# symek/facedeform

Hardware: AMD Instinct MI355X
Metric: deformed Mverts/sec at 256 ctrl pts, 1/2/4/8 MI355X vs host-CPU ref (higher is better)
Workload: dtype f32

## Files before the change

### facedeform_amd/csrc/fd_build_reg.hip

```cpp
#include <cstdio>
#include <cstdlib>

#include "fd_internal.h"
#include "fd_pack.h"

namespace fd {

namespace {

typedef double double4_t __attribute__((ext_vector_type(4)));

constexpr double kEps = 2.220446049250313e-16;
constexpr int kRegThreads = 512;
constexpr int kRegWaves = kRegThreads / 64;
constexpr int kMaxBlocks = 16;
constexpr int kWorkers = 7;
constexpr int kSlots = 20;
constexpr int kPitch = 17;
constexpr int kTileLds = 16 * kPitch;

__device__ __forceinline__ double readlane_f64(double v, int src_lane)
{
    const long long b = __double_as_longlong(v);
    const unsigned lo = (unsigned)__builtin_amdgcn_readlane((int)(b & 0xffffffffll), src_lane);
// ... 52 lines not shown
    return fma(y0, p, y0);
}

__device__ __forceinline__ double log_pos(double x)
{
    double m = __builtin_amdgcn_frexp_mant(x);
    int e = __builtin_amdgcn_frexp_exp(x);
    if (m < 0.70710678118654752) { m *= 2.0; e -= 1; }
    const double num = m - 1.0, den = m + 1.0;
    double r = __builtin_amdgcn_rcp(den);
    r = fma(fma(-den, r, 1.0), r, r);
    r = fma(fma(-den, r, 1.0), r, r);
    double s0 = num * r;
    s0 = fma(fma(-den, s0, num), r, s0);
    const double z = s0 * s0;
    double p = 1.0 / 21.0;
    p = fma(p, z, 1.0 / 19.0);
    p = fma(p, z, 1.0 / 17.0);
    p = fma(p, z, 1.0 / 15.0);
    p = fma(p, z, 1.0 / 13.0);
    p = fma(p, z, 1.0 / 11.0);
    p = fma(p, z, 1.0 / 9.0);
    p = fma(p, z, 1.0 / 7.0);
    p = fma(p, z, 1.0 / 5.0);
    p = fma(p, z, 1.0 / 3.0);
    const double lnm = fma(s0 * z, 2.0 * p, 2.0 * s0);
    return fma((double)e, 0.69314718055994530942, lnm);
}
__device__ __forceinline__ double phi_reg(int kind, double d2, double inv_r2)
{
    switch (kind) {
    case FD_KERNEL_GAUSSIAN: return exp(-d2 * inv_r2);
    case FD_KERNEL_THIN_PLATE: return d2 > 0.0 ? 0.5 * d2 * log_pos(d2) : 0.0;
    case FD_KERNEL_BIHARMONIC: return -sqrt(d2);
    default: return d2 * sqrt(d2);
    }
}

struct RegLds {
    double *cen, *V, *W, *F, *B21, *small, *minv, *P, *scr, *Z, *Y, *stat, *ypart, *D;
    int *tab, *flag;
};
constexpr int kSmallDoubles = 96;
constexpr int kTau = 0, kR = 4, kTm = 20, kG = 36, kGm = 48;
constexpr int kRows = 16 * kMaxBlocks;
__host__ __device__ inline size_t reg_lds_doubles(int)
{
    const size_t overlay = (size_t)kMaxBlocks * kTileLds + (size_t)(kMaxBlocks + 1) * kTileLds;
    const size_t ypart = (size_t)kRegWaves * 4 * kRows;
    return (size_t)3 * kRows + 4 * (size_t)kRows + 4 * (size_t)kRows + 3 * (size_t)kRows + 4 * (size_t)kRows + kSmallDoubles +
           (overlay > ypart ? overlay : ypart) + (size_t)kRegWaves * 2 * kTileLds + 3 * 256 + 3 * 256 + 8 + kTileLds + 160 ;
}
__device__ __forceinline__ RegLds carve(double *base, int)
{
    RegLds L;
    double *p = base;
    L.cen = p; p += 3 * kRows;
    L.V = p; p += 4 * kRows;
    L.W = p; p += 4 * kRows;
    L.F = p; p += 3 * kRows;
    L.B21 = p; p += 4 * kRows;
    L.small = p; p += kSmallDoubles;
    const size_t overlay = (size_t)kMaxBlocks * kTileLds + (size_t)(kMaxBlocks + 1) * kTileLds;
    const size_t ypart = (size_t)kRegWaves * 4 * kRows;
    L.minv = p; L.P = p + (size_t)kMaxBlocks * kTileLds; L.ypart = p;
    p += overlay > ypart ? overlay : ypart;
    L.scr = p; p += (size_t)kRegWaves * 2 * kTileLds;
    L.Z = p; p += 3 * 256;
    L.Y = p; p += 3 * 256;
    L.stat = p; p += 8;
    L.D = p; p += kTileLds;
    L.tab = reinterpret_cast<int *>(p);
    L.flag = L.tab + 300;
    return L;
}

__device__ __forceinline__ double4_t factor_invert_tile(double4_t Tt, int lane, double &piv)
{
    const int c = lane & 15, g = lane >> 4;
    piv = 0.0;
    double4_t U;
#pragma unroll
    for (int i = 0; i < 4; ++i) U[i] = (g + 4 * i == c) ? 1.0 : 0.0;
#pragma unroll
    for (int b = 0; b < 4; ++b) {
        double s[4][4];
#pragma unroll
        for (int p = 0; p < 4; ++p)
#pragma unroll
            for (int q = 0; q <= p; ++q) s[p][q] = readlane_f64(Tt[b], 4 * b + q + 16 * p);
        double l[4][4], inv[4], dk[4];
#pragma unroll
        for (int k = 0; k < 4; ++k) {
            double d = s[k][k];
#pragma unroll
            for (int e = 0; e < k; ++e) d = fma(-l[k][e], l[k][e], d);
            dk[k] = d;
            inv[k] = rsqrt_nr(d);
#pragma unroll
            for (int p = k + 1; p < 4; ++p) {
                double v = s[p][k];
#pragma unroll
                for (int e = 0; e < k; ++e) v = fma(-l[p][e], l[k][e], v);
                l[p][k] = v * inv[k];
            }
        }
#pragma unroll
        for (int k = 0; k < 4; ++k) piv = c == 4 * b + k ? dk[k] : piv;
        double m[4][4];
#pragma unroll
        for (int q = 0; q < 4; ++q) {
            m[q][q] = inv[q];
#pragma unroll
            for (int p = q + 1; p < 4; ++p) {
                double v = 0.0;
#pragma unroll
                for (int e = q; e < p; ++e) v = fma(l[p][e], m[e][q], v);
                m[p][q] = -v * inv[p];
            }
        }
        double aop = 0.0;
#pragma unroll
        for (int p = 0; p < 4; ++p)
#pragma unroll
            for (int q = 0; q <= p; ++q) aop = (c == p && g == q) ? m[p][q] : aop;
        const double4_t zero = {0.0, 0.0, 0.0, 0.0};
        const double4_t rt = __builtin_amdgcn_mfma_f64_16x16x4f64(aop, Tt[b], zero, 0, 0, 0);
        const double4_t ru = __builtin_amdgcn_mfma_f64_16x16x4f64(aop, U[b], zero, 0, 0, 0);
        const double mult = c > 4 * b + 3 ? -rt[0] : 0.0;
        Tt = __builtin_amdgcn_mfma_f64_16x16x4f64(mult, rt[0], Tt, 0, 0, 0);
        U = __builtin_amdgcn_mfma_f64_16x16x4f64(mult, ru[0], U, 0, 0, 0);
        U[b] = ru[0];
        Tt[b] = rt[0];
    }
    return U;
}

constexpr int kAff = 64;
struct PackLds {
    const double *cen, *dlt, *sol, *aff;
    const float *dl_global;
    double R;
    int sing, dup;
    __device__ __forceinline__ double centre(int j, int q) const { return cen[3 * j + q]; }
    __device__ __forceinline__ bool has_delta() const { return true; }
    __device__ __forceinline__ double delta(int j, int q) const { return dlt ? dlt[3 * j + q] : (double)dl_global[3 * j + q]; }
    __device__ __forceinline__ double weight(int j, int c) const { return sol[c * 256 + j]; }
    __device__ __forceinline__ double affine(int cc, int k, int, int T) const { return k < T ? aff[3 * k + cc] : 0.0; }
    __device__ __forceinline__ double radius(int) const { return R; }
    __device__ __forceinline__ int sing_flag() const { return sing; }
    __device__ __forceinline__ int dup_flag() const { return dup; }
};

__device__ __forceinline__ double lds_where(bool cond, const double *p, int i_true)
{
    const double v = p[cond ? i_true : 0];
    return cond ? v : 0.0;
}

__device__ __forceinline__ void assemble_tile(const double *cen, int I, int J, int c, int g, int M, int kind, double lambda, double inv_r2,
                                              double (&e)[4], double &amax_w, bool &dup)
{
    const int col = 16 * J + c;
    const double cx = cen[3 * col], cy = cen[3 * col + 1], cz = cen[3 * col + 2];
    double d2[4];
#pragma unroll
    for (int i = 0; i < 4; ++i) {
        const int row = 16 * I + g + 4 * i;
        const double dx = cen[3 * row] - cx, dy = cen[3 * row + 1] - cy, dz = cen[3 * row + 2] - cz;
        d2[i] = dx * dx + dy * dy + dz * dz;
    }
    if (kind == FD_KERNEL_THIN_PLATE) {
#pragma unroll
        for (int i = 0; i < 4; ++i) {
            const bool pos = d2[i] > 0.0;
            const double lg = log_pos(pos ? d2[i] : 1.0);
            e[i] = pos ? 0.5 * d2[i] * lg : 0.0;
        }
    } else {
#pragma unroll
        for (int i = 0; i < 4; ++i) e[i] = phi_reg(kind, d2[i], inv_r2);
    }
#pragma unroll
    for (int i = 0; i < 4; ++i) {
        const int row = 16 * I + g + 4 * i;
        const bool real = row < M && col < M;
        if (row == col) e[i] += lambda;
        else if (d2[i] == 0.0 && real) dup = true;
        if (!real) e[i] = 0.0;
        const double ae = fabs(e[i]);
        amax_w = ae > amax_w ? ae : amax_w;
    }
}

__device__ __forceinline__ void reflect_wave(const RegLds &L, int M, int T, int lane)
{
    bool singular = false;
    double cn[4] = {0.0, 0.0, 0.0, 0.0};
    double v[4][4], f[4][3];
#pragma unroll
    for (int q = 0; q < 4; ++q) {
        const int i = lane + 64 * q;
        const bool in = i < M;
        const int ic = in ? i : 0;
        const double p[4] = {1.0, L.cen[3 * ic], L.cen[3 * ic + 1], L.cen[3 * ic + 2]};
#pragma unroll
        for (int t = 0; t < 4; ++t) {
            v[q][t] = (in && t < T) ? p[t] : 0.0;
            if (in) cn[t] = fma(v[q][t], v[q][t], cn[t]);
        }
#pragma unroll
        for (int e = 0; e < 3; ++e) { const double d = L.F[e * kRows + ic]; f[q][e] = in ? d : 0.0; }
    }
#pragma unroll
    for (int t = 0; t < 4; ++t) cn[t] = wave_sum(cn[t]);
#pragma unroll
    for (int k = 0; k < 4; ++k) {
        if (k >= T) break;
        const int piv = M - 1 - k;
        const int pl = __builtin_amdgcn_readfirstlane(piv & 63), pq = __builtin_amdgcn_readfirstlane(piv >> 6);
        double rowv[4], rowf[3];
#define FD_PIVOT_ROW(Q) { _Pragma("unroll") for (int t = 0; t < 4; ++t) rowv[t] = readlane_f64(v[Q][t], pl); \
                          _Pragma("unroll") for (int e = 0; e < 3; ++e) rowf[e] = readlane_f64(f[Q][e], pl); }
        if (pq == 0) FD_PIVOT_ROW(0) else if (pq == 1) FD_PIVOT_ROW(1) else if (pq == 2) FD_PIVOT_ROW(2) else FD_PIVOT_ROW(3)
#undef FD_PIVOT_ROW
        double acc[7] = {0.0, 0.0, 0.0, 0.0, 0.0, 0.0, 0.0};
        double x[4];
#pragma unroll
        for (int q = 0; q < 4; ++q) {
            const int i = lane + 64 * q;
            x[q] = i < piv ? v[q][k] : 0.0;
            if (i < piv) {
                acc[0] = fma(x[q], x[q], acc[0]);
#pragma unroll
                for (int cc = k + 1; cc < 4; ++cc) if (cc < T) acc[cc - k] = fma(x[q], v[q][cc], acc[cc - k]);
#pragma unroll
                for (int e = 0; e < 3; ++e) acc[4 + e] = fma(x[q], f[q][e], acc[4 + e]);
            }
        }
#pragma unroll
        for (int e = 0; e < 7; ++e) acc[e] = wave_sum(acc[e]);
        const double xp = rowv[k];
        const double sigma = acc[0];
        const double norm = sqrt(fma(xp, xp, sigma));
        double beta = xp, tau = 0.0, scale = 0.0;
        if (sigma > 0.0) {
            beta = xp >= 0.0 ? -norm : norm;
            tau = (beta - xp) / beta;
            scale = 1.0 / (xp - beta);
        }
        if (!(norm > 64.0 * (double)M * kEps * sqrt(cn[k]))) singular = true;
        double sc[4] = {0.0, 0.0, 0.0, 0.0}, prow[4] = {0.0, 0.0, 0.0, 0.0}, df[3];
#pragma unroll
        for (int cc = k + 1; cc < 4; ++cc) if (cc < T) { prow[cc] = rowv[cc]; sc[cc] = fma(scale, acc[cc - k], prow[cc]); }
#pragma unroll
        for (int e = 0; e < 3; ++e) df[e] = fma(scale, acc[4 + e], rowf[e]);
#pragma unroll
        for (int q = 0; q < 4; ++q) {
            const int i = lane + 64 * q;
            if (i < piv) {
                const double vv = x[q] * scale;
                v[q][k] = vv;
#pragma unroll
                for (int cc = k + 1; cc < 4; ++cc) if (cc < T) v[q][cc] = fma(-tau * sc[cc], vv, v[q][cc]);
#pragma unroll
                for (int e = 0; e < 3; ++e) f[q][e] = fma(-tau * df[e], vv, f[q][e]);
            } else if (i == piv) {
                v[q][k] = 1.0;
#pragma unroll
                for (int cc = k + 1; cc < 4; ++cc) if (cc < T) v[q][cc] = 0.0;
#pragma unroll
                for (int e = 0; e < 3; ++e) f[q][e] = 0.0;
            }
        }
        if (lane == 0) {
            L.small[kTau + k] = tau;
            L.small[kR + 4 * k + k] = beta;
#pragma unroll
            for (int cc = k + 1; cc < 4; ++cc) if (cc < T) L.small[kR + 4 * k + cc] = fma(-tau, sc[cc], prow[cc]);
#pragma unroll
            for (int e = 0; e < 3; ++e) L.small[kG + 3 * k + e] = fma(-tau, df[e], rowf[e]);
        }
    }
#pragma unroll
    for (int q = 0; q < 4; ++q) {
        const int i = lane + 64 * q;
#pragma unroll
        for (int t = 0; t < 4; ++t) L.V[4 * i + t] = v[q][t];
#pragma unroll
        for (int e = 0; e < 3; ++e) L.F[e * kRows + i] = f[q][e];
    }
    wave_lds_sync();
    double gram[6] = {0.0, 0.0, 0.0, 0.0, 0.0, 0.0};
#pragma unroll
    for (int q = 0; q < 4; ++q) {
        const int i = lane + 64 * q;
        if (i < M) {
            const double v0 = v[q][0], v1 = v[q][1], v2 = v[q][2], v3 = v[q][3];
            gram[0] = fma(v0, v1, gram[0]); gram[1] = fma(v0, v2, gram[1]); gram[2] = fma(v0, v3, gram[2]);
            gram[3] = fma(v1, v2, gram[3]); gram[4] = fma(v1, v3, gram[4]); gram[5] = fma(v2, v3, gram[5]);
        }
    }
#pragma unroll
    for (int e = 0; e < 6; ++e) gram[e] = wave_sum(gram[e]);
    {
        const double G[4][4] = {{0.0, gram[0], gram[1], gram[2]}, {0.0, 0.0, gram[3], gram[4]}, {0.0, 0.0, 0.0, gram[5]}, {0.0, 0.0, 0.0, 0.0}};
// ... 730 lines not shown
            L.stat[0] = piv_min; L.stat[1] = piv_max;
            if (bad) L.stat[2] = 1.0;
        }
    }
    FD_RSTAMP()

    auto solve_block = [&](int I) {
        if (lane < 48) {
            const int rhs = lane >> 4, n = lane & 15;
            const double *mi = L.minv + (size_t)I * kTileLds;
            double y = 0.0;
#pragma unroll
            for (int k = 0; k < 16; ++k) y = fma(L.Z[rhs * 256 + 16 * I + k], mi[k * kPitch + n], y);
            L.Y[rhs * 256 + 16 * I + n] = y;
        }
    };
    if (!worker && nb > 0) solve_block(nb - 1);
    __syncthreads();
    if (fac != nullptr && blockIdx.z == 0) {
        gdouble *fg = as_global(fac);
#pragma unroll
        for (int t = 0; t < kSlots; ++t) {
            if (FD_SLOT(m_matrix, t)) {
                const int q = __builtin_amdgcn_readlane(ijv, t) >> 16;
#pragma unroll
                for (int i = 0; i < 4; ++i) fg[kFacL + ((size_t)q * 4 + i) * 64 + lane] = S[t][i];
            }
        }
        for (int e = tid; e < kMaxBlocks * kTileLds; e += kRegThreads) fg[kFacMinv + e] = e < nb * kTileLds ? L.minv[e] : 0.0;
        for (int e = tid; e < 4 * kRows; e += kRegThreads) { fg[kFacV + e] = L.V[e]; fg[kFacB21 + e] = L.B21[e]; }
        if (tid < kSmallDoubles) fg[kFacSmall + tid] = L.small[tid];
        if (tid == 0) {
            fg[kFacMeta + 0] = amax; fg[kFacMeta + 1] = dup_any ? 1.0 : 0.0;
            fg[kFacMeta + 2] = (L.stat[2] != 0.0 || L.stat[3] != 0.0) ? 1.0 : 0.0;
            fg[kFacMeta + 3] = L.stat[0]; fg[kFacMeta + 4] = L.stat[1];
        }
    }
    for (int I = nb - 1; I >= 1; --I) {
        const unsigned m_row = slots_where(ivI == I && ivJ < I);
        const bool next_mine = slots_where(ivI == I && ivJ == I - 1) != 0u;
#pragma unroll
        for (int t = 0; t < kSlots; ++t) {
            if (FD_SLOT(m_row, t)) {
                double4_t acc = {0.0, 0.0, 0.0, 0.0};
                double ya[4];
#pragma unroll
                for (int s = 0; s < 4; ++s) ya[s] = lds_where(c < 3, L.Y, c * 256 + 16 * I + 4 * s + g);
                __builtin_amdgcn_sched_group_barrier(0x100, 4, 0);
                __builtin_amdgcn_sched_group_barrier(0x002, 8, 0);
                __builtin_amdgcn_sched_group_barrier(0x008, 4, 0);
#pragma unroll
                for (int s = 0; s < 4; ++s) acc = __builtin_amdgcn_mfma_f64_16x16x4f64(ya[s], S[t][s], acc, 0, 0, 0);
                if (g < 3) L.Z[g * 256 + 16 * tJ(t) + c] -= acc[0];
            }
        }
        if (next_mine) { wave_lds_sync(); solve_block(I - 1); }
        __syncthreads();
    }
    FD_RSTAMP()

    if (!worker) {
        double q12[12];
#pragma unroll
        for (int e = 0; e < 12; ++e) q12[e] = 0.0;
        double xr[4][3];
#pragma unroll
        for (int q = 0; q < 4; ++q) {
            const int i = lane + 64 * q;
            const bool in = i < n1;
            xr[q][0] = in ? L.Y[i] : 0.0; xr[q][1] = in ? L.Y[256 + i] : 0.0; xr[q][2] = in ? L.Y[512 + i] : 0.0;
            if (in && T > 0) {
#pragma unroll
                for (int k = 0; k < 4; ++k) {
                    const double b = k < T ? L.B21[4 * i + k] : 0.0;
                    q12[3 * k] = fma(b, xr[q][0], q12[3 * k]); q12[3 * k + 1] = fma(b, xr[q][1], q12[3 * k + 1]); q12[3 * k + 2] = fma(b, xr[q][2], q12[3 * k + 2]);
                }
            }
        }
        if (T > 0) {
#pragma unroll
            for (int e = 0; e < 12; ++e) q12[e] = wave_sum(q12[e]);
        }
        double a[4][3] = {};
#pragma unroll
        for (int k = 3; k >= 0; --k) {
            if (k >= T) continue;
#pragma unroll
            for (int e = 0; e < 3; ++e) {
                double v = L.small[kG + 3 * k + e] - q12[3 * k + e];
#pragma unroll
                for (int c2 = k + 1; c2 < 4; ++c2) if (c2 < T) v = fma(-L.small[kR + 4 * k + c2], a[c2][e], v);
                a[k][e] = v / L.small[kR + 4 * k + k];
            }
        }
#pragma unroll
        for (int k = 3; k >= 0; --k) {
            if (k >= T) continue;
            const int piv = M - 1 - k;
            const double tau = L.small[kTau + k];
            double d[3] = {0.0, 0.0, 0.0}, v[4];
#pragma unroll
            for (int q = 0; q < 4; ++q) {
                const int i = lane + 64 * q;
                v[q] = i <= piv ? L.V[4 * i + k] : 0.0;
#pragma unroll
                for (int e = 0; e < 3; ++e) d[e] = fma(v[q], xr[q][e], d[e]);
            }
#pragma unroll
            for (int e = 0; e < 3; ++e) d[e] = wave_sum(d[e]);
#pragma unroll
            for (int q = 0; q < 4; ++q)
#pragma unroll
                for (int e = 0; e < 3; ++e) xr[q][e] = fma(-tau * d[e], v[q], xr[q][e]);
        }
        gdouble *X = as_global(slot.X);
#pragma unroll
        for (int q = 0; q < 4; ++q) {
            const int i = lane + 64 * q;
            if (i < M) { X[i] = xr[q][0]; X[(size_t)npad + i] = xr[q][1]; X[2 * (size_t)npad + i] = xr[q][2]; }
            if (i < M) { L.Y[i] = xr[q][0]; L.Y[256 + i] = xr[q][1]; L.Y[512 + i] = xr[q][2]; }
        }
        if (lane < 12) {
            double v = 0.0;
#pragma unroll
            for (int k = 0; k < 4; ++k)
#pragma unroll
                for (int e = 0; e < 3; ++e) v = lane == 3 * k + e ? a[k][e] : v;
            L.small[kAff + lane] = v;
        }
        for (int r = M + lane; r < npad; r += 64) {
#pragma unroll
            for (int e = 0; e < 3; ++e) {
                double v = 0.0;
#pragma unroll
                for (int k = 0; k < 4; ++k) v = (r - M == k && k < T) ? a[k][e] : v;
                X[(size_t)e * npad + r] = v;
            }
        }
        if (lane == 0) {
            model->terminationtype = 0;
            model->dup_flag = dup_any ? 1 : 0;
            model->sing_flag = (L.stat[2] != 0.0 || L.stat[3] != 0.0) ? 1 : 0;
            L.stat[4] = (L.stat[2] != 0.0 || L.stat[3] != 0.0) ? 1.0 : 0.0;
            L.stat[5] = dup_any ? 1.0 : 0.0;
            model->iterations = M + T;
            model->amax_bits = (unsigned long long)__double_as_longlong(amax);
            model->pivmin_bits = (unsigned long long)__double_as_longlong(L.stat[0]);
            model->pivmax_bits = (unsigned long long)__double_as_longlong(L.stat[1]);
        }
    }
    __threadfence_block();
    __syncthreads();
    FD_RSTAMP()
    if (tid >= 256) return;
    {
        const PackLds in{L.cen, FRONT ? nullptr : L.scr, L.Y, L.small + kAff, slot.delta, gauss_R, L.stat[4] != 0.0 ? 1 : 0, L.stat[5] != 0.0 ? 1 : 0};
        packing::pack_body_from(in, slot, npad, M, Mpad, T, kind, 0, 0);
    }
    FD_RSTAMP()
    if (kind == FD_KERNEL_THIN_PLATE) {
        __syncthreads();
        for (int tile = tid >> 6; tile < Mpad / 16; tile += 4) packing::pack_tiles_body(slot, Mpad, tile, lane);
    }
    FD_RSTAMP()
#undef FD_RSTAMP
#undef tI
#undef tJ
#undef FD_SLOT
}

__global__ __launch_bounds__(256) void k_resolve_reg(const BatchSlot *tab, const PointSrc src, int use_src, int M, int T, int npad, int kind,
                                                      int Mpad, double gauss_R, const double *fac)
{
    const int fi = 1 + (int)blockIdx.z;
    const BatchSlot &slot = tab[fi];
    __shared__ double s_minv[kMaxBlocks * kTileLds];
    __shared__ double s_V[4 * kRows], s_B21[4 * kRows], s_small[kSmallDoubles];
    __shared__ double s_f[3 * kRows];
    __shared__ double s_blk[3 * 16];
    __shared__ double s_red[4 * 12];
    __shared__ double s_g[12], s_a[12];
    const int tid = threadIdx.x, lane = tid & 63;
    const int n1 = M - T, nb = (n1 + 15) / 16, nbk = (M + 15) / 16;
    gcdouble *fg = as_global(fac);
    DevModel FD_GLOBAL *model = as_global(slot.model);
    auto tile_q = [&](int I, int J) { return J * nbk - J * (J - 1) / 2 + (I - J); };
    for (int e = tid; e < kMaxBlocks * kTileLds; e += 256) s_minv[e] = fg[kFacMinv + e];
    for (int e = tid; e < 4 * kRows; e += 256) { s_V[e] = fg[kFacV + e]; s_B21[e] = fg[kFacB21 + e]; }
    if (tid < kSmallDoubles) s_small[tid] = fg[kFacSmall + tid];
    {
        const float *rest = use_src ? src.rest[fi] : slot.rest;
        const float *delta = use_src ? src.delta[fi] : slot.delta;
        for (int i = tid; i < kRows; i += 256) {
#pragma unroll
            for (int q = 0; q < 3; ++q) {
                double d = 0.0;
                if (i < M) {
                    const float r = rest[3 * i + q], dl = delta[3 * i + q];
                    d = (double)dl;
                    slot.centres[3 * i + q] = (double)r;
                    if (use_src) { slot.rest[3 * i + q] = r; slot.delta[3 * i + q] = dl; }
                }
                s_f[q * kRows + i] = d;
            }
            if (i < M) slot.radii[i] = gauss_R;
        }
    }
    __syncthreads();
    const int i0 = tid;
    for (int k = 0; k < T; ++k) {
        const int piv = M - 1 - k;
        const double v = s_V[4 * i0 + k];
        double d[3] = {v * s_f[i0], v * s_f[kRows + i0], v * s_f[2 * kRows + i0]};
        packing::block_reduce_many<3, false>(d, s_red, tid);
        const double tau = s_small[kTau + k];
#pragma unroll
        for (int e = 0; e < 3; ++e) {
            const double fv = fma(-tau * d[e], v, s_f[e * kRows + i0]);
            if (i0 == piv) { s_g[3 * k + e] = fv; s_f[e * kRows + i0] = 0.0; }
            else if (i0 < piv) s_f[e * kRows + i0] = fv;
        }
        __syncthreads();
    }
    {
        const int r = tid, I = r >> 4, rr = r & 15;
        double cur[16], nxt[16];
        auto fetch = [&](int K, double (&dst)[16]) {
            if (I > K && I < nb) {
                gcdouble *p = fg + kFacL + ((size_t)tile_q(I, K) * 4 + (rr >> 2)) * 64 + 16 * (rr & 3);
#pragma unroll
                for (int k = 0; k < 16; ++k) dst[k] = p[k];
            } else {
#pragma unroll
                for (int k = 0; k < 16; ++k) dst[k] = 0.0;
            }
        };
        fetch(0, cur);
        for (int K = 0; K < nb; ++K) {
            if (K + 1 < nb) fetch(K + 1, nxt);
            if (tid < 48) {
                const int e = tid >> 4, n = tid & 15;
                const double *mk = s_minv + (size_t)K * kTileLds;
                double z = 0.0;
#pragma unroll
                for (int k = 0; k < 16; ++k) z = fma(s_f[e * kRows + 16 * K + k], mk[n * kPitch + k], z);
                s_blk[e * 16 + n] = z;
            }
            __syncthreads();
            if (tid < 48) s_f[(tid >> 4) * kRows + 16 * K + (tid & 15)] = s_blk[tid];
            if (I > K && I < nb) {
#pragma unroll
                for (int e = 0; e < 3; ++e) {
                    double acc = s_f[e * kRows + r];
#pragma unroll
                    for (int k = 0; k < 16; ++k) acc = fma(-cur[k], s_blk[e * 16 + k], acc);
                    s_f[e * kRows + r] = acc;
                }
            }
            __syncthreads();
#pragma unroll
            for (int k = 0; k < 16; ++k) cur[k] = nxt[k];
        }
    }
    {
        const int cidx = tid, J = cidx >> 4, cc = cidx & 15;
        double cur[16], nxt[16];
        auto fetch = [&](int I, double (&dst)[16]) {
            if (I > J && I < nb) {
                gcdouble *p = fg + kFacL + (size_t)tile_q(I, J) * 256 + cc;
#pragma unroll
                for (int rr = 0; rr < 16; ++rr) dst[rr] = p[(rr >> 2) * 64 + 16 * (rr & 3)];
            } else {
#pragma unroll
                for (int rr = 0; rr < 16; ++rr) dst[rr] = 0.0;
            }
        };
        if (nb > 0) fetch(nb - 1, cur);
        for (int I = nb - 1; I >= 0; --I) {
            if (I > 0) fetch(I - 1, nxt);
            if (tid < 48) {
                const int e = tid >> 4, n = tid & 15;
                const double *mi = s_minv + (size_t)I * kTileLds;
                double y = 0.0;
#pragma unroll
                for (int k = 0; k < 16; ++k) y = fma(s_f[e * kRows + 16 * I + k], mi[k * kPitch + n], y);
                s_blk[e * 16 + n] = y;
            }
            __syncthreads();
            if (tid < 48) s_f[(tid >> 4) * kRows + 16 * I + (tid & 15)] = s_blk[tid];
            if (J < I) {
#pragma unroll
                for (int e = 0; e < 3; ++e) {
                    double acc = s_f[e * kRows + cidx];
#pragma unroll
                    for (int rr = 0; rr < 16; ++rr) acc = fma(-cur[rr], s_blk[e * 16 + rr], acc);
                    s_f[e * kRows + cidx] = acc;
                }
            }
            __syncthreads();
#pragma unroll
            for (int rr = 0; rr < 16; ++rr) cur[rr] = nxt[rr];
        }
    }
    double xr[3];
    {
        const bool in = i0 < n1;
#pragma unroll
        for (int e = 0; e < 3; ++e) xr[e] = in ? s_f[e * kRows + i0] : 0.0;
        double q12[12];
#pragma unroll
        for (int k = 0; k < 4; ++k) {
            const double b = (in && k < T) ? s_B21[4 * i0 + k] : 0.0;
#pragma unroll
            for (int e = 0; e < 3; ++e) q12[3 * k + e] = b * xr[e];
        }
        if (T > 0) packing::block_reduce_many<12, false>(q12, s_red, tid);
        if (tid == 0) {
            double a[4][3] = {};
#pragma unroll
            for (int k = 3; k >= 0; --k) {
                if (k >= T) continue;
#pragma unroll
                for (int e = 0; e < 3; ++e) {
                    double v = s_g[3 * k + e] - q12[3 * k + e];
#pragma unroll
                    for (int c2 = k + 1; c2 < 4; ++c2) if (c2 < T) v = fma(-s_small[kR + 4 * k + c2], a[c2][e], v);
                    a[k][e] = v / s_small[kR + 4 * k + k];
                }
            }
#pragma unroll
            for (int k = 0; k < 4; ++k)
#pragma unroll
                for (int e = 0; e < 3; ++e) s_a[3 * k + e] = a[k][e];
        }
        for (int k = T - 1; k >= 0; --k) {
            const int piv = M - 1 - k;
            const double v = i0 <= piv ? s_V[4 * i0 + k] : 0.0;
            double d[3] = {v * xr[0], v * xr[1], v * xr[2]};
            packing::block_reduce_many<3, false>(d, s_red, tid);
            const double tau = s_small[kTau + k];
#pragma unroll
            for (int e = 0; e < 3; ++e) xr[e] = fma(-tau * d[e], v, xr[e]);
        }
        __syncthreads();
        gdouble *X = as_global(slot.X);
        if (i0 < M) { X[i0] = xr[0]; X[(size_t)npad + i0] = xr[1]; X[2 * (size_t)npad + i0] = xr[2]; }
        for (int rrow = M + tid; rrow < npad; rrow += 256) {
#pragma unroll
            for (int e = 0; e < 3; ++e) X[(size_t)e * npad + rrow] = (rrow - M < T) ? s_a[3 * (rrow - M) + e] : 0.0;
        }
        if (tid == 0) {
            model->terminationtype = 0;
            model->dup_flag = fg[kFacMeta + 1] != 0.0 ? 1 : 0;
            model->sing_flag = fg[kFacMeta + 2] != 0.0 ? 1 : 0;
            model->iterations = M + T;
            model->amax_bits = (unsigned long long)__double_as_longlong(fg[kFacMeta + 0]);
            model->pivmin_bits = (unsigned long long)__double_as_longlong(fg[kFacMeta + 3]);
            model->pivmax_bits = (unsigned long long)__double_as_longlong(fg[kFacMeta + 4]);
        }
    }
    __threadfence_block();
    __syncthreads();
    packing::pack_body(slot, npad, M, Mpad, T, kind, 0, 0);
    if (kind == FD_KERNEL_THIN_PLATE) {
        __syncthreads();
        for (int tile = tid >> 6; tile < Mpad / 16; tile += 4) packing::pack_tiles_body(slot, Mpad, tile, lane);
    }
}

}

size_t reg_factor_doubles() { return kFacDoubles; }

bool reg_applicable(int kind, int term, double lambda, int M)
{
    return M <= 16 * kMaxBlocks && spd_applicable(kind, term, lambda, M);
}

hipError_t reg_build_init()
{
    static bool done[64] = {};
    int dev = 0;
    hipError_t e = hipGetDevice(&dev);
    if (e != hipSuccess) return e;
    if (dev >= 0 && dev < 64 && done[dev]) return hipSuccess;
    e = hipFuncSetAttribute((const void *)k_build_reg<true>, hipFuncAttributeMaxDynamicSharedMemorySize,
                            (int)(sizeof(double) * reg_lds_doubles(16 * kMaxBlocks)));
    if (e == hipSuccess)
        e = hipFuncSetAttribute((const void *)k_build_reg<false>, hipFuncAttributeMaxDynamicSharedMemorySize,
                                (int)(sizeof(double) * reg_lds_doubles(16 * kMaxBlocks)));
    if (e == hipSuccess && dev >= 0 && dev < 64) done[dev] = true;
    return e;
}

hipError_t launch_build_reg_shared(const BuildBuffers &b, hipStream_t stream, const PointSrc *src, hipEvent_t ev_mid, double *fac)
{
    static const PointSrc none{};
    if (ev_mid) (void)hipEventRecord(ev_mid, stream);
    const size_t lds = sizeof(double) * reg_lds_doubles(b.M);
    hipLaunchKernelGGL(k_build_reg<true>, dim3(1, 1, 1), dim3(kRegThreads), lds, stream, b.d_slots, src ? *src : none, src ? 1 : 0, b.M, b.T,
                       b.npad, b.kind, b.Mpad, b.lambda, b.gauss_R, (unsigned long long *)nullptr, fac);
    if (b.nbatch > 1)
        hipLaunchKernelGGL(k_resolve_reg, dim3(1, 1, (unsigned)b.nbatch - 1), dim3(256), 0, stream, b.d_slots, src ? *src : none, src ? 1 : 0,
                           b.M, b.T, b.npad, b.kind, b.Mpad, b.gauss_R, (const double *)fac);
    return hipGetLastError();
}

hipError_t launch_build_reg(const BuildBuffers &b, hipStream_t stream, const PointSrc *src, hipEvent_t ev_mid)
{
    static const PointSrc none{};
    const unsigned nbatch = (unsigned)b.nbatch;
    if (ev_mid) (void)hipEventRecord(ev_mid, stream);
    const size_t lds = sizeof(double) * reg_lds_doubles(b.M);
    static unsigned long long *d_stamps = nullptr;
    hipStreamCaptureStatus cs = hipStreamCaptureStatusNone;
    static const bool stamps_env = tuning_env("FD_REG_STAMPS") != nullptr;
    static const bool stamps_late = stamps_env && atoi(tuning_env("FD_REG_STAMPS")) == 2;
    const bool want_stamps = stamps_env && hipStreamIsCapturing(stream, &cs) == hipSuccess && cs == hipStreamCaptureStatusNone;
    if (want_stamps && !d_stamps) { (void)hipMalloc((void **)&d_stamps, 96 * sizeof(unsigned long long)); (void)hipMemset(d_stamps, 0, 96 * sizeof(unsigned long long)); }
    const bool split = b.reg_front != 0 && reg_front_doubles(b.M) <= ns_doubles(b.M);
    if (split) {
        const int nbk = (b.M + 15) / 16, ntiles = nbk * (nbk + 1) / 2;
        const int cus = (int)device_cus();
        auto tiles_per_wave = [&](int per_wg) {
            int tpw = 1;
            while (tpw < kFrontMaxTpw && ((ntiles + per_wg * tpw - 1) / (per_wg * tpw)) * (int)nbatch > cus) ++tpw;
            return tpw;
        };
        const int tpw1 = tiles_per_wave(kFront1Tiles), tpw2 = tiles_per_wave(kFront2Tiles);
        hipLaunchKernelGGL(k_reg_front1, dim3((unsigned)((ntiles + kFront1Tiles * tpw1 - 1) / (kFront1Tiles * tpw1)), 1, nbatch), dim3(kRegThreads), 0, stream,
                           b.d_slots, src ? *src : none, src ? 1 : 0, b.M, b.T, b.kind, b.lambda, b.gauss_R, tpw1);
        hipLaunchKernelGGL(k_reg_front2, dim3((unsigned)((ntiles + kFront2Tiles * tpw2 - 1) / (kFront2Tiles * tpw2)), 1, nbatch), dim3(kRegThreads), 0, stream,
                           b.d_slots, b.M, b.T, tpw2);
        hipLaunchKernelGGL(k_build_reg<false>, dim3(1, 1, nbatch), dim3(kRegThreads), lds, stream, b.d_slots, none, 0, b.M, b.T,
                           b.npad, b.kind, b.Mpad, b.lambda, b.gauss_R, want_stamps ? d_stamps : nullptr, (double *)nullptr);
    } else
    hipLaunchKernelGGL(k_build_reg<true>, dim3(1, 1, nbatch), dim3(kRegThreads), lds, stream, b.d_slots, src ? *src : none, src ? 1 : 0, b.M, b.T,
                       b.npad, b.kind, b.Mpad, b.lambda, b.gauss_R, want_stamps ? d_stamps : nullptr, (double *)nullptr);
    if (want_stamps && d_stamps && stamps_late) {
        static bool registered = false;
        static unsigned long long *d_keep = nullptr;
        d_keep = d_stamps;
        if (!registered) {
            registered = true;
            atexit([] {
                unsigned long long h[96];
                if (d_keep && hipDeviceSynchronize() == hipSuccess && hipMemcpy(h, d_keep, sizeof(h), hipMemcpyDeviceToHost) == hipSuccess && h[83]) {
                    fprintf(stderr, "[k_build_reg stamps, MEAN over %llu launches (no read-back per launch): table | assembly | tile loads | reflectors | KV | W + rotation | Cholesky | back substitution | recovery | pack]\n  ", h[83]);
                    for (int q = 0; q < 10; ++q) fprintf(stderr, " %llu", h[84 + q] / h[83]);
                    fprintf(stderr, "\n");
                }
            });
        }
    } else if (want_stamps && d_stamps) {
        unsigned long long h[80];
        (void)hipStreamSynchronize(stream);
        if (hipMemcpy(h, d_stamps, sizeof(h), hipMemcpyDeviceToHost) == hipSuccess) {
            fprintf(stderr, "[k_build_reg stamps, shader cycles: table | assembly | tile loads | reflectors + Q^T f | Y = K V | W + rotation + B21 | Cholesky | back substitution | recovery | pack]\n  ");
            for (int q = 0; q < 10; ++q) fprintf(stderr, " %llu", h[q]);
            fprintf(stderr, "\n   Cholesky steps (cycles since its start: inverse K in LDS | panel K in LDS, as wave 0 sees them):");
            for (int q = 16; q < 48; ++q) fprintf(stderr, "%s%llu", (q - 16) % 2 ? " " : "\n     ", h[q]);
            fprintf(stderr, "\n");
        }
    }
    return hipGetLastError();
}

}
```

### facedeform_amd/csrc/fd_pack.h

```cpp
#pragma once

#include "fd_internal.h"

namespace fd {
namespace packing {

__device__ __forceinline__ double block_sum(double v, double *scratch, int tid)
{
    for (int off = 32; off >= 1; off >>= 1) v += __shfl_xor(v, off);
    __syncthreads();
    if ((tid & 63) == 0) scratch[tid >> 6] = v;
    __syncthreads();
    return scratch[0] + scratch[1] + scratch[2] + scratch[3];
}
__device__ __forceinline__ double block_max(double v, double *scratch, int tid)
{
    for (int off = 32; off >= 1; off >>= 1) { const double o = __shfl_xor(v, off); v = o > v ? o : v; }
    __syncthreads();
    if ((tid & 63) == 0) scratch[tid >> 6] = v;
    __syncthreads();
    const double a = scratch[0] > scratch[1] ? scratch[0] : scratch[1];
    const double b = scratch[2] > scratch[3] ? scratch[2] : scratch[3];
    return a > b ? a : b;
}
// ... 82 lines not shown
    for (int j = tid; j < M; j += 256) {
        const double x = in.centre(j, 0), y = in.centre(j, 1), z = in.centre(j, 2);
        const double d = (x - cenx) * (x - cenx) + (y - ceny) * (y - ceny) + (z - cenz) * (z - cenz);
        r2 = d > r2 ? d : r2;
        const double o = x * x + y * y + z * z;
        r2o = o > r2o ? o : r2o;
        if (dl) {
            const double a = in.delta(j, 0), b = in.delta(j, 1), c2 = in.delta(j, 2);
            const double dd = a * a + b * b + c2 * c2;
            dmax2 = dd > dmax2 ? dd : dmax2;
            ndmin2 = -dd > ndmin2 ? -dd : ndmin2;
        }
    }
    double ext[4] = {r2, r2o, dmax2, ndmin2};
    block_reduce_many<4, true>(ext, s_red, tid);
    if (dl) {
        const double moving2 = 1e-2 * ext[2];
        double nmin[1] = {-INFINITY};
        for (int j = tid; j < M; j += 256) {
            const double a = in.delta(j, 0), b = in.delta(j, 1), c2 = in.delta(j, 2);
            const double dd = a * a + b * b + c2 * c2;
            if (dd >= moving2 && dd > 0.0 && -dd > nmin[0]) nmin[0] = -dd;
        }
        block_reduce_many<1, true>(nmin, s_red, tid);
        ext[3] = nmin[0] > -INFINITY ? nmin[0] : 0.0;
    }
    const double rad_c = sqrt(ext[0]);
    const double rad_o = sqrt(ext[1]);
    const double cen = sqrt(cenx * cenx + ceny * ceny + cenz * cenz);
    double x0[3] = {0.0, 0.0, 0.0};
    double rad = rad_o;
    if (cen > rad_c * 0.0625) { x0[0] = (double)(float)cenx; x0[1] = (double)(float)ceny; x0[2] = (double)(float)cenz; rad = rad_c; }
    double sc = 1.0;
    if (rad > 0.0 && isfinite(rad)) {
        int e = (int)rint(log2(rad));
        e = e < -100 ? -100 : (e > 100 ? 100 : e);
        sc = ldexp(1.0, e);
    }
    const double inv_s = 1.0 / sc;
    double w32 = 1.0, w64 = 1.0, kappa = 0.0;
    if (kind == FD_KERNEL_THIN_PLATE) { w32 = 0.5 * kLn2 * sc * sc; w64 = 0.5; kappa = sc * sc * log(sc); }
    if (kind == FD_KERNEL_BIHARMONIC) { w32 = -sc; w64 = -1.0; }
    if (kind == FD_KERNEL_CUBIC) { w32 = sc * sc * sc; }

    bool bad = false;
    float wmax = 0.f;
    double m[18];
#pragma unroll
    for (int q = 0; q < 18; ++q) m[q] = 0.0;
    for (int j = tid; j < Mpad; j += 256) {
        Rec32 r32 = {0.f, 0.f, 0.f, 0.f, 0.f, 0.f, 0.f, 0.f};
        Rec64 r64 = {0.0, 0.0, 0.0, 0.0, 0.0, 0.0, 0.0, 0.0};
        if (j < M) {
            const double w[3] = {in.weight(j, 0), in.weight(j, 1), in.weight(j, 2)};
            bad |= !(isfinite(w[0]) && isfinite(w[1]) && isfinite(w[2]));
            if (!from_w) { W[3 * j] = w[0]; W[3 * j + 1] = w[1]; W[3 * j + 2] = w[2]; }
            const double R = in.radius(j);
            r64.cx = in.centre(j, 0); r64.cy = in.centre(j, 1); r64.cz = in.centre(j, 2);
            r64.s = gauss ? -1.0 / (R * R) : 0.0;
            r64.wx = w[0] * w64; r64.wy = w[1] * w64; r64.wz = w[2] * w64;
            const double cn[3] = {(r64.cx - x0[0]) * inv_s, (r64.cy - x0[1]) * inv_s, (r64.cz - x0[2]) * inv_s};
            r32.cx = (float)cn[0]; r32.cy = (float)cn[1]; r32.cz = (float)cn[2];
            r32.s = gauss ? (float)(-kLog2e * sc * sc / (R * R)) : 0.f;
            r32.wx = (float)(w[0] * w32); r32.wy = (float)(w[1] * w32); r32.wz = (float)(w[2] * w32);
            wmax = fmaxf(wmax, fmaxf(fabsf(r32.wx), fmaxf(fabsf(r32.wy), fabsf(r32.wz))));
            const double cc2 = cn[0] * cn[0] + cn[1] * cn[1] + cn[2] * cn[2];
#pragma unroll
            for (int c = 0; c < 3; ++c) {
                m[5 * c] += w[c];
                m[5 * c + 1] += w[c] * cn[0];
                m[5 * c + 2] += w[c] * cn[1];
                m[5 * c + 3] += w[c] * cn[2];
                m[5 * c + 4] += w[c] * cc2;
                m[15 + c] += fabs(w[c] * w32);
            }
        }
        int jo = j;
        if (layers > 1 && j < M) { const int Mc = M / layers; jo = (j % Mc) * layers + j / Mc; }
        rec32[jo] = r32;
        rec64[jo] = r64;
    }
    block_reduce_many<18, false>(m, s_red, tid);
    double wm[1] = {(double)wmax};
    block_reduce_many<1, true>(wm, s_red, tid);

    __shared__ double s_aff[12];
    if (tid < 12) {
        const int cc = tid / 4, k = tid % 4;
        const double v = in.affine(cc, k, M, T);
        bad |= !isfinite(v);
        if (!from_w) W[3 * (M + k) + cc] = v;
        model->affine64[tid] = v;
        s_aff[tid] = v;
    }
    if (bad) s_bad = 1;
    __syncthreads();
    float pmax = 0.f;
    if (tid < 3) {
        const int c = tid;
        const double *a = s_aff + 4 * c;
        const float p5[5] = {(float)(a[0] + a[1] * x0[0] + a[2] * x0[1] + a[3] * x0[2] + kappa * m[5 * c + 4]),
                             (float)(a[1] * sc - 2.0 * kappa * m[5 * c + 1]), (float)(a[2] * sc - 2.0 * kappa * m[5 * c + 2]),
                             (float)(a[3] * sc - 2.0 * kappa * m[5 * c + 3]), (float)(kappa * m[5 * c])};
#pragma unroll
        for (int e = 0; e < 5; ++e) { model->poly32[5 * c + e] = p5[e]; pmax = fmaxf(pmax, fabsf(p5[e])); }
        model->norm32[c] = (float)x0[c];
    }
    pmax = fmaxf(pmax, fmaxf(__shfl(pmax, 1), __shfl(pmax, 2)));
    if (tid == 0) {
        model->wmax32 = fmaxf((float)wm[0], pmax);
        const double phimax = kind == FD_KERNEL_THIN_PLATE ? 8.0 : (kind == FD_KERNEL_CUBIC ? 8.0 : (kind == FD_KERNEL_BIHARMONIC ? 2.0 : 1.0));
        double S = 0.0;
#pragma unroll
        for (int c = 0; c < 3; ++c) {
            const double *a = s_aff + 4 * c;
            const double poly = fabs(a[0]) + (fabs(a[1]) + fabs(a[2]) + fabs(a[3])) * (rad_o > 0.0 ? rad_o : 1.0) + 4.0 * fabs(kappa * m[5 * c]);
            const double v = m[15 + c] * phimax + poly;
            S = v > S ? v : S;
        }
        const double dmax = sqrt(ext[2]), dmin = dl ? sqrt(-ext[3]) : 0.0;
        model->fp32_error = S * 2.98023223876953125e-08;
        model->cancellation = dmax > 0.0 ? S / dmax : 0.0;
        model->delta_min = dmin;
        model->delta_max = dmax;
        model->extent = rad_o;
        model->norm32[3] = (float)inv_s;
        int tt = 1;
        if (from_w == 1) {
            if (s_bad) tt = -4;
        } else {
            if (in.sing_flag() || s_bad) tt = -4;
            if (in.dup_flag()) tt = -5;
        }
        model->terminationtype = tt;
        if (slot.host_status) *slot.host_status = tt;
    }
}

__device__ __forceinline__ void pack_body(const BatchSlot &slot, int npad, int M, int Mpad, int T, int kind, int from_w, int layers)
{
    const PackGlobal in{from_w ? nullptr : slot.X, slot.W, slot.centres, slot.radii, from_w ? nullptr : slot.delta, slot.model, npad, from_w};
    pack_body_from(in, slot, npad, M, Mpad, T, kind, from_w, layers);
}

__device__ __forceinline__ void split3_bf16(float x, unsigned &hi, unsigned &mid, unsigned &lo)
{
    const unsigned u = __float_as_uint(x);
    const float r1 = x - __uint_as_float(u & 0xffff0000u);
    const unsigned u1 = __float_as_uint(r1);
    const float r2 = r1 - __uint_as_float(u1 & 0xffff0000u);
    hi = u >> 16; mid = u1 >> 16; lo = __float_as_uint(r2) >> 16;
}

__device__ __forceinline__ void pack_tiles_body(const BatchSlot &slot, int Mpad, int tile, int lane)
{
    const Rec32 *rec32 = slot.rec32;
    MfmaTile *tiles = slot.tiles;
    const int g = lane >> 4, i = lane & 15;
    const Rec32 r = rec32[16 * tile + i];
    unsigned h, m, l;
    unsigned k[8] = {0, 0, 0, 0, 0, 0, 0, 0};
    if (g < 3) {
        const float c = g == 0 ? r.cx : (g == 1 ? r.cy : r.cz);
        split3_bf16(c, h, m, l);
        k[0] = h; k[1] = h; k[2] = m; k[3] = m; k[4] = h; k[5] = l;
    } else {
        const float cc = fmaf(r.cz, r.cz, fmaf(r.cy, r.cy, r.cx * r.cx));
        split3_bf16(cc, h, m, l);
        k[0] = h; k[1] = m; k[2] = l;
        k[3] = 0x3f80; k[4] = 0x3f80; k[5] = 0x3f80;
    }
    MfmaTile &t = tiles[tile];
    t.a[lane][0] = k[0] | (k[1] << 16);
    t.a[lane][1] = k[2] | (k[3] << 16);
    t.a[lane][2] = k[4] | (k[5] << 16);
    t.a[lane][3] = k[6] | (k[7] << 16);
    if (i < 12) {
        const int pair = i / 6, c = (i % 6) / 2, half = i % 2;
        const Rec32 rw = rec32[16 * tile + 4 * g + 2 * pair + half];
        t.w[g][i] = c == 0 ? rw.wx : (c == 1 ? rw.wy : rw.wz);
    }
    if (lane < 16) t.pad[lane] = 0.f;
    (void)Mpad;

    MfmaTileH *tiles16 = slot.tiles16;
    if (tiles16) {
        MfmaTileH &th = tiles16[tile];
        const float v = g < 3 ? (g == 0 ? r.cx : (g == 1 ? r.cy : r.cz)) : fmaf(r.cz, r.cz, fmaf(r.cy, r.cy, r.cx * r.cx));
        const _Float16 vh = (_Float16)v;
        const _Float16 vl = (_Float16)(v - (float)vh);
        const unsigned uh = (unsigned)__builtin_bit_cast(unsigned short, vh), ul = (unsigned)__builtin_bit_cast(unsigned short, vl);
        if (g < 3) { th.a[lane][0] = uh | (uh << 16); th.a[lane][1] = ul | (ul << 16); }
        else { th.a[lane][0] = uh | (ul << 16); th.a[lane][1] = 0x3c003c00u; }
        if (i < 12) th.w[g][i] = t.w[g][i];
        if (lane < 16) th.pad[lane] = 0.f;
    }
}

}
}
```

Measured before the change: 63880.

## Rewrite regression packing epilogue to use all 512 threads with fewer barriers

Replaces the generic pack_body_from epilogue, which ran on only 256 threads, with a specialised pack_reg that keeps all 8 waves busy. The two 4-wave halves split the reductions between them, and reductions use wave butterflies plus LDS scratch placed in the inverse-block region. Record images are staged in LDS so the MFMA tile packing reads them from LDS instead of global memory, and that packing is spread over 7 waves. This targets the serial tail of the build kernel; the metric is dominated by deformation throughput, so the effect may be small, and the rewrite risks numerical or layout mismatches with the old packer.

```diff
diff --git a/facedeform_amd/csrc/fd_build_reg.hip b/facedeform_amd/csrc/fd_build_reg.hip
--- a/facedeform_amd/csrc/fd_build_reg.hip
+++ b/facedeform_amd/csrc/fd_build_reg.hip
@@ -228,6 +228,231 @@
     __device__ __forceinline__ int dup_flag() const { return dup; }
 };
 
+constexpr int kPkCen = 0, kPkExt = 12, kPkR2 = 20, kPkNmin = 24, kPkMom = 32, kPkWm = 104, kPkAff = 108, kPkBad = 120, kPkRec = 128;
+constexpr int kPkDoubles = kPkRec + kRows * (int)(sizeof(Rec32) / sizeof(double));
+static_assert(kPkDoubles <= kMaxBlocks * kTileLds, "the packing's scratch lies in the inverse blocks' LDS");
+__device__ __forceinline__ void bfly_sum(double &v)
+{
+    for (int off = 32; off >= 1; off >>= 1) v += __shfl_xor(v, off);
+}
+__device__ __forceinline__ void bfly_max(double &v)
+{
+    for (int off = 32; off >= 1; off >>= 1) { const double o = __shfl_xor(v, off); v = o > v ? o : v; }
+}
+__device__ __forceinline__ double sum4(const double *p, int stride) { return p[0] + p[stride] + p[2 * stride] + p[3 * stride]; }
+__device__ __forceinline__ double max4(const double *p, int stride)
+{
+    const double a = p[0] > p[stride] ? p[0] : p[stride];
+    const double b = p[2 * stride] > p[3 * stride] ? p[2 * stride] : p[3 * stride];
+    return a > b ? a : b;
+}
+
+template <class Stamp>
+__device__ __forceinline__ void pack_reg(const PackLds &in, const BatchSlot &slot, int M, int Mpad, int T, int kind, double *scr, Stamp stamp)
+{
+    const int tid = threadIdx.x, lane = tid & 63;
+    const int wave = __builtin_amdgcn_readfirstlane(tid >> 6);
+    const bool hi = wave >= 4;
+    const int wq = wave & 3;
+    const int j = tid & 255;
+    const bool rec = j < M;
+    gdouble *W = as_global(slot.W);
+    Rec32 FD_GLOBAL *rec32 = as_global(slot.rec32);
+    Rec64 FD_GLOBAL *rec64 = as_global(slot.rec64);
+    DevModel FD_GLOBAL *model = as_global(slot.model);
+    int *s_bad = reinterpret_cast<int *>(scr + kPkBad);
+    Rec32 *rimg = reinterpret_cast<Rec32 *>(scr + kPkRec);
+    const double kLn2 = 0.6931471805599453;
+    const double kLog2e = 1.4426950408889634;
+    const bool gauss = kind == FD_KERNEL_GAUSSIAN || kind == FD_KERNEL_GAUSSIAN_QNN;
+    double x = 0.0, y = 0.0, z = 0.0, da = 0.0, db = 0.0, dc = 0.0;
+    if (rec) { x = in.centre(j, 0); y = in.centre(j, 1); z = in.centre(j, 2); }
+    if (hi && rec) { da = in.delta(j, 0); db = in.delta(j, 1); dc = in.delta(j, 2); }
+    if (tid == 0) *s_bad = 0;
+
+    if (!hi) {
+        double s[3] = {0.0, 0.0, 0.0};
+        if (rec) { s[0] += x; s[1] += y; s[2] += z; }
+#pragma unroll
+        for (int q = 0; q < 3; ++q) bfly_sum(s[q]);
+        if (lane == 0) { scr[kPkCen + wq] = s[0]; scr[kPkCen + 4 + wq] = s[1]; scr[kPkCen + 8 + wq] = s[2]; }
+    } else {
+        double r2o = 0.0, dmax2 = 0.0;
+        if (rec) {
+            const double o = x * x + y * y + z * z;
+            r2o = o > r2o ? o : r2o;
+            const double dd = da * da + db * db + dc * dc;
+            dmax2 = dd > dmax2 ? dd : dmax2;
+        }
+        bfly_max(r2o);
+        bfly_max(dmax2);
+        if (lane == 0) { scr[kPkExt + wq] = r2o; scr[kPkExt + 4 + wq] = dmax2; }
+    }
+    __syncthreads();
+    const double cenx = sum4(scr + kPkCen, 1) / M, ceny = sum4(scr + kPkCen + 4, 1) / M, cenz = sum4(scr + kPkCen + 8, 1) / M;
+    const double r2o = max4(scr + kPkExt, 1), dmax2 = max4(scr + kPkExt + 4, 1);
+
+    if (!hi) {
+        double r2 = 0.0;
+        if (rec) {
+            const double d = (x - cenx) * (x - cenx) + (y - ceny) * (y - ceny) + (z - cenz) * (z - cenz);
+            r2 = d > r2 ? d : r2;
+        }
+        bfly_max(r2);
+        if (lane == 0) scr[kPkR2 + wq] = r2;
+    } else {
+        const double moving2 = 1e-2 * dmax2;
+        double nmin = -INFINITY;
+        if (rec) {
+            const double dd = da * da + db * db + dc * dc;
+            if (dd >= moving2 && dd > 0.0 && -dd > nmin) nmin = -dd;
+        }
+        bfly_max(nmin);
+        if (lane == 0) scr[kPkNmin + wq] = nmin;
+        if (wave == 4 && lane < 12) {
+            const int cc = lane / 4, k = lane % 4;
+            const double v = in.affine(cc, k, M, T);
+            W[3 * (M + k) + cc] = v;
+            model->affine64[lane] = v;
+            scr[kPkAff + lane] = v;
+            if (!isfinite(v)) *s_bad = 1;
+        }
+    }
+    __syncthreads();
+    const double r2 = max4(scr + kPkR2, 1);
+    double nmin = max4(scr + kPkNmin, 1);
+    nmin = nmin > -INFINITY ? nmin : 0.0;
+    const double rad_c = sqrt(r2);
+    const double rad_o = sqrt(r2o);
+    const double cen = sqrt(cenx * cenx + ceny * ceny + cenz * cenz);
+    double x0[3] = {0.0, 0.0, 0.0};
+    double rad = rad_o;
+    if (cen > rad_c * 0.0625) { x0[0] = (double)(float)cenx; x0[1] = (double)(float)ceny; x0[2] = (double)(float)cenz; rad = rad_c; }
+    double sc = 1.0;
+    if (rad > 0.0 && isfinite(rad)) {
+        int e = (int)rint(log2(rad));
+        e = e < -100 ? -100 : (e > 100 ? 100 : e);
+        sc = ldexp(1.0, e);
+    }
+    const double inv_s = 1.0 / sc;
+    double w32 = 1.0, w64 = 1.0;
+    if (kind == FD_KERNEL_THIN_PLATE) { w32 = 0.5 * kLn2 * sc * sc; w64 = 0.5; }
+    if (kind == FD_KERNEL_BIHARMONIC) { w32 = -sc; w64 = -1.0; }
+    if (kind == FD_KERNEL_CUBIC) { w32 = sc * sc * sc; }
+    stamp();
+
+    double w[3] = {0.0, 0.0, 0.0}, cn[3] = {0.0, 0.0, 0.0}, cc2 = 0.0;
+    if (rec) {
+        w[0] = in.weight(j, 0); w[1] = in.weight(j, 1); w[2] = in.weight(j, 2);
+        cn[0] = (x - x0[0]) * inv_s; cn[1] = (y - x0[1]) * inv_s; cn[2] = (z - x0[2]) * inv_s;
+        cc2 = cn[0] * cn[0] + cn[1] * cn[1] + cn[2] * cn[2];
+    }
+    auto moment = [&](int q) -> double {
+        if (!rec) return 0.0;
+        const int c = q < 15 ? q / 5 : q - 15, k = q % 5;
+        const double t = q >= 15 ? fabs(w[c] * w32) : (k == 0 ? w[c] : (k == 4 ? w[c] * cc2 : w[c] * cn[k - 1]));
+        return 0.0 + t;
+    };
+    if (!hi) {
+        Rec32 r32 = {0.f, 0.f, 0.f, 0.f, 0.f, 0.f, 0.f, 0.f};
+        Rec64 r64 = {0.0, 0.0, 0.0, 0.0, 0.0, 0.0, 0.0, 0.0};
+        bool bad = false;
+        float wmax = 0.f;
+        if (rec) {
+            bad = !(isfinite(w[0]) && isfinite(w[1]) && isfinite(w[2]));
+            W[3 * j] = w[0]; W[3 * j + 1] = w[1]; W[3 * j + 2] = w[2];
+            const double R = in.radius(j);
+            r64.cx = x; r64.cy = y; r64.cz = z;
+            r64.s = gauss ? -1.0 / (R * R) : 0.0;
+            r64.wx = w[0] * w64; r64.wy = w[1] * w64; r64.wz = w[2] * w64;
+            r32.cx = (float)cn[0]; r32.cy = (float)cn[1]; r32.cz = (float)cn[2];
+            r32.s = gauss ? (float)(-kLog2e * sc * sc / (R * R)) : 0.f;
+            r32.wx = (float)(w[0] * w32); r32.wy = (float)(w[1] * w32); r32.wz = (float)(w[2] * w32);
+            wmax = fmaxf(wmax, fmaxf(fabsf(r32.wx), fmaxf(fabsf(r32.wy), fabsf(r32.wz))));
+        }
+        if (j < Mpad) {
+            typedef float f32x4 __attribute__((ext_vector_type(4)));
+            f32x4 FD_GLOBAL *g32 = (f32x4 FD_GLOBAL *)(rec32 + j);
+            double4_t FD_GLOBAL *g64 = (double4_t FD_GLOBAL *)(rec64 + j);
+            g32[0] = (f32x4){r32.cx, r32.cy, r32.cz, r32.s}; g32[1] = (f32x4){r32.wx, r32.wy, r32.wz, r32.pad};
+            g64[0] = (double4_t){r64.cx, r64.cy, r64.cz, r64.s}; g64[1] = (double4_t){r64.wx, r64.wy, r64.wz, r64.pad};
+            rimg[j] = r32;
+        }
+        if (bad) *s_bad = 1;
+        double m[9];
+#pragma unroll
+        for (int q = 0; q < 9; ++q) m[q] = moment(q);
+        double wm = (double)wmax;
+#pragma unroll
+        for (int q = 0; q < 9; ++q) bfly_sum(m[q]);
+        bfly_max(wm);
+        if (lane == 0) {
+#pragma unroll
+            for (int q = 0; q < 9; ++q) scr[kPkMom + 18 * wq + q] = m[q];
+            scr[kPkWm + wq] = wm;
+        }
+    } else {
+        double m[9];
+#pragma unroll
+        for (int q = 0; q < 9; ++q) m[q] = moment(9 + q);
+#pragma unroll
+        for (int q = 0; q < 9; ++q) bfly_sum(m[q]);
+        if (lane == 0) {
+#pragma unroll
+            for (int q = 0; q < 9; ++q) scr[kPkMom + 18 * wq + 9 + q] = m[q];
+        }
+    }
+    __syncthreads();
+    stamp();
+
+    if (wave == 0) {
+        const double *mom = scr + kPkMom;
+        const double *s_aff = scr + kPkAff;
+        double kappa = 0.0;
+        if (kind == FD_KERNEL_THIN_PLATE) kappa = sc * sc * log(sc);
+        float pmax = 0.f;
+        if (tid < 3) {
+            const int c = tid;
+            const double *a = s_aff + 4 * c;
+            const double m0 = sum4(mom + 5 * c, 18), m1x = sum4(mom + 5 * c + 1, 18), m1y = sum4(mom + 5 * c + 2, 18);
+            const double m1z = sum4(mom + 5 * c + 3, 18), m2 = sum4(mom + 5 * c + 4, 18);
+            const float p5[5] = {(float)(a[0] + a[1] * x0[0] + a[2] * x0[1] + a[3] * x0[2] + kappa * m2),
+                                 (float)(a[1] * sc - 2.0 * kappa * m1x), (float)(a[2] * sc - 2.0 * kappa * m1y),
+                                 (float)(a[3] * sc - 2.0 * kappa * m1z), (float)(kappa * m0)};
+#pragma unroll
+            for (int e = 0; e < 5; ++e) { model->poly32[5 * c + e] = p5[e]; pmax = fmaxf(pmax, fabsf(p5[e])); }
+            model->norm32[c] = (float)(c == 0 ? x0[0] : (c == 1 ? x0[1] : x0[2]));
+        }
+        pmax = fmaxf(pmax, fmaxf(__shfl(pmax, 1), __shfl(pmax, 2)));
+        if (tid == 0) {
+            model->wmax32 = fmaxf((float)max4(scr + kPkWm, 1), pmax);
+            const double phimax = kind == FD_KERNEL_THIN_PLATE ? 8.0 : (kind == FD_KERNEL_CUBIC ? 8.0 : (kind == FD_KERNEL_BIHARMONIC ? 2.0 : 1.0));
+            double S = 0.0;
+#pragma unroll
+            for (int c = 0; c < 3; ++c) {
+                const double *a = s_aff + 4 * c;
+                const double poly = fabs(a[0]) + (fabs(a[1]) + fabs(a[2]) + fabs(a[3])) * (rad_o > 0.0 ? rad_o : 1.0) + 4.0 * fabs(kappa * sum4(mom + 5 * c, 18));
+                const double v = sum4(mom + 15 + c, 18) * phimax + poly;
+                S = v > S ? v : S;
+            }
+            const double dmax = sqrt(dmax2), dmin = sqrt(-nmin);
+            model->fp32_error = S * 2.98023223876953125e-08;
+            model->cancellation = dmax > 0.0 ? S / dmax : 0.0;
+            model->delta_min = dmin;
+            model->delta_max = dmax;
+            model->extent = rad_o;
+            model->norm32[3] = (float)inv_s;
+            int tt = 1;
+            if (in.sing_flag() || *s_bad) tt = -4;
+            if (in.dup_flag()) tt = -5;
+            model->terminationtype = tt;
+            if (slot.host_status) *as_global(slot.host_status) = tt;
+        }
+    } else if (kind == FD_KERNEL_THIN_PLATE) {
+        for (int tile = wave - 1; tile < Mpad / 16; tile += kRegWaves - 1) packing::pack_tiles_body_from(rimg, slot, Mpad, tile, lane);
+    }
+}
+
 __device__ __forceinline__ double lds_where(bool cond, const double *p, int i_true)
 {
     const double v = p[cond ? i_true : 0];
@@ -1264,16 +1489,11 @@
     __threadfence_block();
     __syncthreads();
     FD_RSTAMP()
-    if (tid >= 256) return;
     {
         const PackLds in{L.cen, FRONT ? nullptr : L.scr, L.Y, L.small + kAff, slot.delta, gauss_R, L.stat[4] != 0.0 ? 1 : 0, L.stat[5] != 0.0 ? 1 : 0};
-        packing::pack_body_from(in, slot, npad, M, Mpad, T, kind, 0, 0);
-    }
-    FD_RSTAMP()
-    if (kind == FD_KERNEL_THIN_PLATE) {
-        __syncthreads();
-        for (int tile = tid >> 6; tile < Mpad / 16; tile += 4) packing::pack_tiles_body(slot, Mpad, tile, lane);
-    }
+        pack_reg(in, slot, M, Mpad, T, kind, L.minv, [&]() { FD_RSTAMP() });
+    }
+    if (stamps) __syncthreads();
     FD_RSTAMP()
 #undef FD_RSTAMP
 #undef tI
@@ -1558,8 +1778,8 @@
             atexit([] {
                 unsigned long long h[96];
                 if (d_keep && hipDeviceSynchronize() == hipSuccess && hipMemcpy(h, d_keep, sizeof(h), hipMemcpyDeviceToHost) == hipSuccess && h[83]) {
-                    fprintf(stderr, "[k_build_reg stamps, MEAN over %llu launches (no read-back per launch): table | assembly | tile loads | reflectors | KV | W + rotation | Cholesky | back substitution | recovery | pack]\n  ", h[83]);
-                    for (int q = 0; q < 10; ++q) fprintf(stderr, " %llu", h[84 + q] / h[83]);
+                    fprintf(stderr, "[k_build_reg stamps, MEAN over %llu launches (no read-back per launch): table | assembly | tile loads | reflectors | KV | W + rotation | Cholesky | back substitution | recovery | pack: scale | pack: records, moments | pack: status, tiles]\n  ", h[83]);
+                    for (int q = 0; q < 11; ++q) fprintf(stderr, " %llu", h[84 + q] / h[83]);
                     fprintf(stderr, "\n");
                 }
             });
@@ -1568,8 +1788,8 @@
         unsigned long long h[80];
         (void)hipStreamSynchronize(stream);
         if (hipMemcpy(h, d_stamps, sizeof(h), hipMemcpyDeviceToHost) == hipSuccess) {
-            fprintf(stderr, "[k_build_reg stamps, shader cycles: table | assembly | tile loads | reflectors + Q^T f | Y = K V | W + rotation + B21 | Cholesky | back substitution | recovery | pack]\n  ");
-            for (int q = 0; q < 10; ++q) fprintf(stderr, " %llu", h[q]);
+            fprintf(stderr, "[k_build_reg stamps, shader cycles: table | assembly | tile loads | reflectors + Q^T f | Y = K V | W + rotation + B21 | Cholesky | back substitution | recovery | pack: scale | pack: records, moments | pack: status, tiles]\n  ");
+            for (int q = 0; q < 11; ++q) fprintf(stderr, " %llu", h[q]);
             fprintf(stderr, "\n   Cholesky steps (cycles since its start: inverse K in LDS | panel K in LDS, as wave 0 sees them):");
             for (int q = 16; q < 48; ++q) fprintf(stderr, "%s%llu", (q - 16) % 2 ? " " : "\n     ", h[q]);
             fprintf(stderr, "\n");
diff --git a/facedeform_amd/csrc/fd_pack.h b/facedeform_amd/csrc/fd_pack.h
--- a/facedeform_amd/csrc/fd_pack.h
+++ b/facedeform_amd/csrc/fd_pack.h
@@ -258,10 +258,9 @@
     hi = u >> 16; mid = u1 >> 16; lo = __float_as_uint(r2) >> 16;
 }
 
-__device__ __forceinline__ void pack_tiles_body(const BatchSlot &slot, int Mpad, int tile, int lane)
-{
-    const Rec32 *rec32 = slot.rec32;
-    MfmaTile *tiles = slot.tiles;
+__device__ __forceinline__ void pack_tiles_body_from(const Rec32 *rec32, const BatchSlot &slot, int Mpad, int tile, int lane)
+{
+    MfmaTile FD_GLOBAL *tiles = as_global(slot.tiles);
     const int g = lane >> 4, i = lane & 15;
     const Rec32 r = rec32[16 * tile + i];
     unsigned h, m, l;
@@ -276,7 +275,7 @@
         k[0] = h; k[1] = m; k[2] = l;
         k[3] = 0x3f80; k[4] = 0x3f80; k[5] = 0x3f80;
     }
-    MfmaTile &t = tiles[tile];
+    MfmaTile FD_GLOBAL &t = tiles[tile];
     t.a[lane][0] = k[0] | (k[1] << 16);
     t.a[lane][1] = k[2] | (k[3] << 16);
     t.a[lane][2] = k[4] | (k[5] << 16);
@@ -289,9 +288,9 @@
     if (lane < 16) t.pad[lane] = 0.f;
     (void)Mpad;
 
-    MfmaTileH *tiles16 = slot.tiles16;
+    MfmaTileH FD_GLOBAL *tiles16 = as_global(slot.tiles16);
     if (tiles16) {
-        MfmaTileH &th = tiles16[tile];
+        MfmaTileH FD_GLOBAL &th = tiles16[tile];
         const float v = g < 3 ? (g == 0 ? r.cx : (g == 1 ? r.cy : r.cz)) : fmaf(r.cz, r.cz, fmaf(r.cy, r.cy, r.cx * r.cx));
         const _Float16 vh = (_Float16)v;
         const _Float16 vl = (_Float16)(v - (float)vh);
@@ -302,6 +301,10 @@
         if (lane < 16) th.pad[lane] = 0.f;
     }
 }
-
-}
-}
+__device__ __forceinline__ void pack_tiles_body(const BatchSlot &slot, int Mpad, int tile, int lane)
+{
+    pack_tiles_body_from(slot.rec32, slot, Mpad, tile, lane);
+}
+
+}
+}
```

After: 65660, median of 6. 1.03x the previous value.
